# chongkuiqi/S2ANet

Hardware: AMD Instinct MI355X
Metric: 1024x1024 DOTA chips/sec (R-50-FPN S2ANet inference) (higher is better)
Workload: dtype f16; 1 GPU; BASELINE configs[2]: full R-50-FPN S2ANet inference, batch 8 of 1024x1024 synthetic uint8 chips per GPU; 3 independent batches in flight on 3 HIP streams; global_batch=8, num_classes=15, weights=seeded random init of the reference architecture; odm_cls bias calibrated, nms_candidate_cap=160000, nms_candidates_dropped=0, distinct_input_batches=3, fam_cls_branch=True, hip_graph=False, batches_in_flight=3, parallelism=dp1 (one process per GPU)

## Files before the change

include/s2anet_hip.h:

```cpp
#ifndef S2ANET_HIP_H_
#define S2ANET_HIP_H_

#include <stddef.h>
#include <stdint.h>

#ifdef __cplusplus
extern "C" {
#endif

#define S2A_OK 0
#define S2A_EINVAL (-1)
#define S2A_EWORKSPACE (-2)
#define S2A_EHIP (-3)
#define S2A_ENOTIMPL (-4)

#define S2A_DTYPE_F32 0
#define S2A_DTYPE_F16 1
#define S2A_DTYPE_F64 2

#define S2A_LAYOUT_NCHW 0
#define S2A_LAYOUT_NHWC 1

typedef void* s2a_stream_t;

// ... 194 lines not shown
int s2a_deform_conv_backward(int dtype, const void* input, const void* offset, const void* grad_output, const void* weight,
                             float* grad_input_f32, void* grad_offset, float* grad_weight_f32, float scale, int64_t batch,
                             int64_t channels, int64_t height, int64_t width, int64_t out_channels, void* workspace,
                             size_t workspace_bytes, s2a_stream_t stream);
int s2a_deform_conv_backward_typed(int dtype, const void* input, const void* offset, const void* grad_output,
                                   const void* weight, void* grad_input, void* grad_offset, float* grad_weight_f32,
                                   float scale, int64_t batch, int64_t channels, int64_t height, int64_t width,
                                   int64_t out_channels, void* workspace, size_t workspace_bytes, s2a_stream_t stream);

int s2a_conv3x3_tail1x1_f16(const void* x, const void* weight_frag, const void* bias, const void* tail_weight_frag,
                            const void* tail_bias, const void* residual, void* out, const void* chain_weight_frag,
                            const void* chain_bias, void* chain_out, int64_t chain_channels, int64_t batch, int64_t channels,
                            int64_t mid_channels, int64_t out_channels, int64_t height, int64_t width,
                            s2a_stream_t stream);

int s2a_conv1x1_add_up2_f16(const void* x, const void* weight_frag, const void* bias, const void* coarse,
                            void* out, int64_t batch, int64_t channels, int64_t height, int64_t width,
                            int64_t out_channels, s2a_stream_t stream);

int64_t s2a_pyramid_pixels(const s2a_pyramid* pyr, int64_t batch);
int s2a_conv3x3_pyramid_f16(const void* x, const void* weight_frag, const void* bias, const void* residual,
                            void* out, int64_t batch, int64_t channels, int64_t out_channels, int relu,
                            const s2a_pyramid* pyr, s2a_stream_t stream);
int s2a_conv3x3_head_pyramid_f16(const void* x, const void* weight_frag, const void* bias, void* out,
                                 const void* head_weight_frag, const void* head_bias, void* head_out,
                                 int64_t batch, int64_t channels, int64_t out_channels, int relu,
                                 const s2a_pyramid* pyr, s2a_stream_t stream);
int s2a_orconv_pool_pyramid_f16(const void* x, const void* weight_frag, const void* bias, void* out, void* pooled,
                                int64_t batch, int64_t channels, int64_t out_channels, const s2a_pyramid* pyr,
                                s2a_stream_t stream);
int64_t s2a_conv_wino_packed_elems(int64_t out_channels, int64_t channels);
int s2a_conv_wino_pack_weight_f16(const void* weight, int64_t out_channels, int64_t channels, void* packed,
                                  s2a_stream_t stream);
int s2a_conv3x3_wino_pyramid_f16(const void* x, const void* weight_wino, const void* bias, void* out, void* pooled,
                                 int64_t batch, int64_t channels, int64_t out_channels, int relu,
                                 const s2a_pyramid* pyr, s2a_stream_t stream);
int s2a_align_conv_pyramid_f16(const void* x, const float* anchors, const void* weight_packed, void* out,
                               int64_t batch, int64_t channels, int64_t out_channels, int relu,
                               const s2a_pyramid* pyr, s2a_stream_t stream);
int s2a_fam_refine_anchors_pyramid(const void* pred, int64_t row_stride, int64_t batch, const s2a_pyramid* pyr,
                                   float anchor_scale, float* refined, s2a_stream_t stream);

int64_t s2a_stem_packed_elems(void);
int s2a_stem_pack_weight_f16(const void* weight, void* packed, s2a_stream_t stream);
int s2a_stem_u8_f16(const void* image_u8, const void* weight_packed, const void* bias, void* out,
                    int64_t batch, int64_t height, int64_t width, float divisor, s2a_stream_t stream);
// ... 46 lines not shown
```

s2anet_amd/_lib.py:

```python
import ctypes
import os
import subprocess

import torch

_HERE = os.path.dirname(os.path.abspath(__file__))
LIB_PATH = os.environ.get("S2A_LIB_PATH") or os.path.join(_HERE, "libs2anet_hip.so")

OK, EINVAL, EWORKSPACE, EHIP, ENOTIMPL = 0, -1, -2, -3, -4
DTYPE_F32, DTYPE_F16, DTYPE_F64 = 0, 1, 2
LAYOUT_NCHW, LAYOUT_NHWC = 0, 1

c_i64, c_int, c_f32, c_sz, c_vp = (ctypes.c_int64, ctypes.c_int, ctypes.c_float, ctypes.c_size_t,
                                   ctypes.c_void_p)


class DcnParams(ctypes.Structure):
    _fields_ = [("batch", c_i64), ("channels", c_i64), ("height", c_i64), ("width", c_i64),
                ("out_channels", c_i64),
                ("kW", c_int), ("kH", c_int), ("dW", c_int), ("dH", c_int), ("padW", c_int),
                ("padH", c_int), ("dilationW", c_int), ("dilationH", c_int), ("group", c_int),
                ("deformable_group", c_int), ("dtype", c_int), ("offset_dtype", c_int),
                ("layout", c_int), ("relu", c_int)]

# ... 89 lines not shown
    "s2a_deform_conv_backward_weight_workspace_bytes": (c_sz, [c_i64, c_i64, c_i64, c_i64, c_i64]),
    "s2a_deform_conv_backward_workspace_bytes": (c_sz, [c_int, c_i64, c_i64, c_i64, c_i64, c_i64]),
    "s2a_deform_conv_backward": (c_int, [c_int, c_vp, c_vp, c_vp, c_vp, c_vp, c_vp, c_vp, c_f32, c_i64, c_i64, c_i64, c_i64,
                                         c_i64, c_vp, c_sz, c_vp]),
    "s2a_deform_conv_backward_typed": (c_int, [c_int, c_vp, c_vp, c_vp, c_vp, c_vp, c_vp, c_vp, c_f32, c_i64, c_i64, c_i64, c_i64,
                                               c_i64, c_vp, c_sz, c_vp]),
    "s2a_deform_conv_backward_input_f32_workspace_bytes": (c_sz, [c_i64, c_i64, c_i64, c_i64, c_i64]),
    "s2a_deform_conv_backward_weight_f32_workspace_bytes": (c_sz, [c_i64, c_i64, c_i64, c_i64, c_i64]),
    "s2a_deform_conv_backward_weight_f32": (c_int, [c_vp, c_vp, c_vp, c_vp, c_f32, c_i64, c_i64, c_i64, c_i64, c_i64,
                                                    c_vp, c_sz, c_vp]),
    "s2a_deform_conv_backward_input_f32": (c_int, [c_vp, c_vp, c_vp, c_vp, c_vp, c_vp, c_i64, c_i64, c_i64, c_i64, c_i64,
                                                   c_vp, c_sz, c_vp]),
    "s2a_deform_conv_backward_weight_f16": (c_int, [c_vp, c_vp, c_vp, c_vp, c_i64, c_i64, c_i64, c_i64, c_i64, c_vp, c_sz, c_vp]),
    "s2a_deform_conv_backward_input_f16": (c_int, [c_vp, c_vp, c_vp, c_vp, c_vp, c_vp, c_i64, c_i64, c_i64, c_i64, c_i64,
                                           c_vp, c_sz, c_vp]),
    "s2a_deformable_im2col": (c_int, [c_vp, c_vp, c_vp, ctypes.POINTER(DcnParams), c_vp]),
    "s2a_deformable_col2im": (c_int, [c_vp, c_vp, c_vp, ctypes.POINTER(DcnParams), c_vp]),
    "s2a_deformable_col2im_coord": (c_int, [c_vp, c_vp, c_vp, c_vp, ctypes.POINTER(DcnParams), c_vp]),
    "s2a_conv3x3_tail1x1_f16": (c_int, [c_vp] * 10 + [c_i64] * 7 + [c_vp]),
    "s2a_conv1x1_add_up2_f16": (c_int, [c_vp, c_vp, c_vp, c_vp, c_vp, c_i64, c_i64, c_i64, c_i64, c_i64, c_vp]),
    "s2a_pyramid_pixels": (c_i64, [ctypes.POINTER(Pyramid), c_i64]),
    "s2a_conv3x3_pyramid_f16": (c_int, [c_vp, c_vp, c_vp, c_vp, c_vp, c_i64, c_i64, c_i64, c_int,
                                        ctypes.POINTER(Pyramid), c_vp]),
    "s2a_conv3x3_head_pyramid_f16": (c_int, [c_vp, c_vp, c_vp, c_vp, c_vp, c_vp, c_vp, c_i64, c_i64, c_i64, c_int,
                                             ctypes.POINTER(Pyramid), c_vp]),
    "s2a_orconv_pool_pyramid_f16": (c_int, [c_vp, c_vp, c_vp, c_vp, c_vp, c_i64, c_i64, c_i64, ctypes.POINTER(Pyramid), c_vp]),
    "s2a_conv_wino_packed_elems": (c_i64, [c_i64, c_i64]),
    "s2a_conv_wino_pack_weight_f16": (c_int, [c_vp, c_i64, c_i64, c_vp, c_vp]),
    "s2a_conv3x3_wino_pyramid_f16": (c_int, [c_vp, c_vp, c_vp, c_vp, c_vp, c_i64, c_i64, c_i64, c_int,
                                             ctypes.POINTER(Pyramid), c_vp]),
    "s2a_align_conv_pyramid_f16": (c_int, [c_vp, c_vp, c_vp, c_vp, c_i64, c_i64, c_i64, c_int,
                                           ctypes.POINTER(Pyramid), c_vp]),
    "s2a_fam_refine_anchors_pyramid": (c_int, [c_vp, c_i64, c_i64, ctypes.POINTER(Pyramid), c_f32, c_vp, c_vp]),
    "s2a_stem_packed_elems": (c_i64, []),
    "s2a_stem_pack_weight_f16": (c_int, [c_vp, c_vp, c_vp]),
    "s2a_stem_u8_f16": (c_int, [c_vp, c_vp, c_vp, c_vp, c_i64, c_i64, c_i64, c_f32, c_vp]),
    "s2a_pyramid_candidates_count": (c_i64, [ctypes.POINTER(Pyramid), c_i64]),
    "s2a_pyramid_candidates": (c_int, [c_vp, c_vp, c_vp, c_i64, ctypes.POINTER(Pyramid), c_int, c_i64, c_f32, c_vp, c_vp, c_vp, c_vp]),
    "s2a_rbox_to_poly": (c_int, [c_vp, c_i64, c_i64, c_vp, c_vp]),
    "s2a_scene_gather_u8": (c_int, [c_vp, c_i64, c_i64, c_vp, c_i64, ctypes.c_int32, c_vp, c_vp]),
    "s2a_scene_merge_workspace_bytes": (c_sz, [c_i64, c_i64]),
    "s2a_scene_merge": (c_int, [c_vp, c_vp, c_vp, c_vp, c_vp, c_i64, c_i64, ctypes.c_int32, ctypes.c_double, c_i64,
                                c_vp, c_vp, c_vp, c_vp, c_vp, c_vp, c_vp, c_sz, c_vp]),
    "s2a_delta2bbox_rotated": (c_int, [c_vp, c_vp, c_i64, c_f32, c_vp, c_vp]),
    "s2a_fam_refine_anchors": (c_int, [c_vp, c_i64, c_i64, c_i64, c_f32, c_f32, c_int, c_int,
                                       c_vp, c_vp]),
# ... 78 lines not shown
```

s2anet_amd/csrc/dcn_ops.hip:

```cpp
#include <hip/hip_fp16.h>
#include <hip/hip_runtime.h>

#include <algorithm>
#include <cstdlib>
#include <cstring>

#include "common.hpp"

namespace s2a {
namespace {

#ifndef S2A_ABL
#define S2A_ABL 0
#endif
#ifndef S2A_STAMP
#define S2A_STAMP 0
#endif
#ifdef S2A_MEASURE
#define S2A_DCN_DROP_SWITCH(xb, wb)                     \
  do {                                                  \
    const char* drop = getenv("S2A_DCN_DROP");          \
    if (drop && strchr(drop, 'x')) (xb) = 0;            \
    if (drop && strchr(drop, 'w')) (wb) = 0;            \
  } while (0)
// ... 1074 lines not shown
  }
  dcn_patch_tile<OUT_NHWC, SRC, TH>(a.x, a.src, a.wfrag, a.out, a.Ntot, a.C, a.H, a.W, a.O, a.stride, a.relu, a.x_bytes, a.lt,
                                        a.tile_base, blockIdx.x, a.n_full ? a.n_full : gridDim.x, threadIdx.x);
}

constexpr int kCPW = 18;

struct ConvExtra {
  _Float16* pool_out;
  const _Float16* head_w;
  const _Float16* head_b;
  _Float16* head_out;
  int store_main;
  const _Float16* tail_w;
  const _Float16* tail_b;
  const _Float16* tail_res;
  _Float16* tail_out;
  const _Float16* chain_w;
  const _Float16* chain_b;
  _Float16* chain_out;
  int chain_O;
};

template <int TAPS, int OG, int PH = 1, int SD = 1, bool TAIL = false, int HT = 0>
struct ConvCfg {
  static constexpr int kTH = (SD == 2 || HT) ? 4 : 8 * PH;
  static constexpr int kPos = (SD == 2 || HT) ? 64 : 128 * PH;
  static constexpr int kWaves = 4 * PH;
  static constexpr int kPW = SD == 2 ? 33 : kCPW;
  static constexpr int kNT = (kPos / 32) * OG / 4 / PH;
  static constexpr int kPix = TAPS == 9 ? ((kTH - 1) * SD + 3) * kPW : kPos;
  static constexpr int kDma = (kPix * 9 + 63) / 64;
  static constexpr int kPatchBytes = kDma * 1024;
  static constexpr int kOutRowB = OG * 128 + 16;
  static constexpr bool kWLds = PH == 2 && TAPS == 9;
  static constexpr int kWBuf = OG * 8192;
  static constexpr int kLoop0 = 2 * kPatchBytes + (kWLds ? 2 * kWBuf : 0);
  static constexpr int kLoop = (kWLds && OG == 1 && kPatchBytes + 9 * 8192 > kLoop0) ? kPatchBytes + 9 * 8192 : kLoop0;
  static constexpr int kLds0 = (kLoop > kPos * kOutRowB) ? kLoop : kPos * kOutRowB;
  static constexpr int kTailRowB = 528;
  static constexpr int kLds = (TAIL && kPos * kTailRowB > kLds0) ? kPos * kTailRowB : kLds0;
  static constexpr int kBiasBytes = TAIL ? 1024 : 512;
  static constexpr int kJ = (kDma + kWaves - 1) / kWaves;
};

template <int TAPS, int OG, int PH = 1, int SD = 1, bool TAIL = false, int HT = 0>
__global__ __launch_bounds__(256 * PH, PH == 1 ? 2 : 1) void k_conv_f16(const _Float16* __restrict__ x_,
                                                     const _Float16* __restrict__ wfrag,
                                                     const _Float16* __restrict__ bias,
                                                     const _Float16* __restrict__ residual_,
                                                     _Float16* __restrict__ out_, int64_t Ntot_, int C,
                                                     int H_, int W_, int Ho_, int Wo_, int cstride, int O,
                                                     int relu, unsigned x_bytes_, LevelTab lt, int res_up,
                                                     ConvExtra ex) {
  _Float16* pool_out_ = ex.pool_out;
  using T = _Float16;
  using V = f16x8;
  using Cfg = ConvCfg<TAPS, OG, PH, SD, TAIL, HT>;
  constexpr int NT = Cfg::kNT;
  static_assert(NT >= 1, "unsupported tile / group combination");
  static_assert(!HT || (TAPS == 9 && PH == 1 && SD == 1 && !TAIL), "half tiles: plain 3x3 / stride 1");
  static_assert(!TAIL || (TAPS == 9 && OG == 1 && SD == 1), "the fused 1x1 tail follows a 64-map 3x3/s1");
  constexpr int WPG = 4 / OG;
  constexpr int kThreads_ = 256 * PH;
  extern __shared__ __attribute__((aligned(16))) char smem[];
  const int tid = threadIdx.x, lane = tid & 63, wave = tid >> 6;
  const int wave4 = wave & 3, blk = wave >> 2;
  int64_t tile = xcd_remap(blockIdx.x, gridDim.x);
  const T* x = x_;
  const T* residual = residual_;
  T* out = out_;
  int64_t Ntot = Ntot_;
  int H = H_, W = W_, Ho = Ho_, Wo = Wo_;
  unsigned x_bytes = x_bytes_;
  if (TAPS == 9 && lt.n > 1) {
    int t0 = 0, p0 = 0;
#pragma unroll
    for (int i = 0; i < kMaxLevels; i++)
      if (i < lt.n && tile >= lt.tile0[i]) {
        t0 = lt.tile0[i]; p0 = lt.pix0[i]; H = lt.H[i]; W = lt.W[i];
      }
    tile -= t0;
    Ho = H; Wo = W;
    Ntot = (int64_t)lt.batch * H * W;
    x += (int64_t)p0 * C;
// ... 48 lines not shown
  }
  auto patch_issue = [&](int cc) {
    char* P = smem + (cc & 1) * Cfg::kPatchBytes;
#pragma unroll
    for (int j = 0; j < Cfg::kJ; j++) {
      const int i = wave_u + Cfg::kWaves * j;
      if (i < Cfg::kDma)
        __builtin_amdgcn_raw_ptr_buffer_load_lds(rx, (__attribute__((address_space(3))) void*)(P + i * 1024), 16,
                                                 (int)pvoff[j], cc * 128, 0, 0);
    }
  };

  const int grp = wave4 / WPG, sub = wave4 % WPG;
  const bool wave_active = grp * 64 < Oloc;
  const int g = min(o0 / 64 + grp, G - 1);
  const V* wf_base = reinterpret_cast<const V*>(wfrag) + lane;
  V wA[2][4], wB[2][4];
  constexpr bool M16 = (TAPS == 9 && SD == 1) || (TAPS == 1 && OG == 4);
  constexpr int NB16 = 2 * NT;
  auto load_w = [&](int s, V (&wv)[2][4]) {
    if constexpr (M16) {
      const V* p = reinterpret_cast<const V*>(wfrag) + ((int64_t)s * G + g) * 8 * 64 + ((lane >> 4) & 1) * 128 + (lane >> 5) * 32 + (lane & 15);
#pragma unroll
      for (int f = 0; f < 8; f++) wv[f >> 2][f & 3] = p[((f >> 2) * 4 + (f & 1)) * 64 + ((f >> 1) & 1) * 16];
      return;
    }
    const V* p = wf_base + ((int64_t)s * G + g) * 8 * 64;
#pragma unroll
    for (int a = 0; a < 2; a++)
#pragma unroll
      for (int kk = 0; kk < 4; kk++) wv[a][kk] = p[(a * 4 + kk) * 64];
  };
  const int lp = (TAPS == 9 && SD == 1) ? ((lane & 16) | (((lane & 15) - ((lane >> 3) & 2)) & 15)) : (lane & 31);
  int fbase[NT];
#pragma unroll
  for (int b = 0; b < NT; b++) {
    int pl = 128 * blk + 32 * (sub * NT + b) + lp;
    int pix = TAPS == 9 ? SD * ((pl >> 4) * Cfg::kPW + (pl & 15)) : pl;
    fbase[b] = pix * kRowBytes + (lane >> 5) * 16;
  }
  f32x16 acc[2][NT];
  f32x4 acc16[M16 ? 4 : 1][M16 ? NB16 : 1];
  if constexpr (M16) {
#pragma unroll
    for (int a = 0; a < 4; a++)
#pragma unroll
      for (int b = 0; b < NB16; b++)
// ... 5 lines not shown
#pragma unroll
      for (int b = 0; b < NT; b++)
#pragma unroll
        for (int r = 0; r < 16; r++) acc[a][b][r] = 0.f;
  }
  const int kg16 = lane >> 4, i16 = lane & 15;
  const int pix16 = (i16 >= 4 && i16 < 12) ? (((i16 - 4) >> 1) * 4 + (i16 & 1))
                                           : (((i16 & 3) >> 1) * 4 + 2 + (i16 & 1) + (i16 >= 12 ? 8 : 0));
  const int t16 = 2 * sub * NT;
  const int fbase16 = (TAPS == 9 ? (8 * blk + t16) * Cfg::kPW + pix16 : 128 * blk + 16 * t16 + pix16) * kRowBytes + (kg16 & 1) * 64 + (kg16 >> 1) * 16;
  constexpr int kTile16 = (TAPS == 9 ? Cfg::kPW : 16) * kRowBytes;
  const int abase16 = (kg16 & 1) * 2048 + ((kg16 >> 1) * 32 + i16) * 16;

  auto compute = [&](const char* P, int t, const V (&wv)[2][4]) {
    if (!wave_active) return;
    const int toff = ((t / 3) * Cfg::kPW + (t % 3)) * kRowBytes;
    if constexpr (M16) {
#pragma unroll
      for (int ks = 0; ks < 2; ks++) {
        V pf[NB16];
#pragma unroll
        for (int b = 0; b < NB16; b++) pf[b] = *reinterpret_cast<const V*>(P + fbase16 + b * kTile16 + toff + ks * 32);
#pragma unroll
        for (int a = 0; a < 4; a++)
#pragma unroll
          for (int b = 0; b < NB16; b++)
            acc16[a][b] = __builtin_amdgcn_mfma_f32_16x16x32_f16(wv[(a * 2 + ks) >> 2][(a * 2 + ks) & 3], pf[b], acc16[a][b], 0, 0, 0);
      }
      return;
    }
#pragma unroll
    for (int kk = 0; kk < 4; kk++) {
      V pf[NT];
#pragma unroll
      for (int b = 0; b < NT; b++) pf[b] = *reinterpret_cast<const V*>(P + fbase[b] + toff + kk * 32);
#pragma unroll
      for (int a = 0; a < 2; a++)
#pragma unroll
        for (int b = 0; b < NT; b++)
          acc[a][b] = __builtin_amdgcn_mfma_f32_32x32x16_f16(wv[a][kk], pf[b], acc[a][b], 0, 0, 0);
    }
  };

  constexpr bool kEarlyRes = TAIL && Cfg::kWLds;
  constexpr int NI2 = TAIL ? Cfg::kPos * 32 / kThreads_ : 1;
  unsigned off2[NI2];
  V r2[NI2];
  auto tail_res_issue = [&]() {
    const __amdgpu_buffer_rsrc_t rr = __builtin_amdgcn_make_buffer_rsrc(
        const_cast<T*>(ex.tail_res ? ex.tail_res : ex.tail_out), 0, (int)((uint64_t)Ntot * 256 * 2), 0x00020000);
#pragma unroll
    for (int i = 0; i < NI2; i++) {
      const int idx = tid + kThreads_ * i, pos = idx >> 5, col = idx & 31;
      const int64_t gp = tile_pos(tile, pos, Cfg::kTH, Ho, Wo, HWo, Ntot);
      off2[i] = gp >= 0 ? (unsigned)((gp * 256 + col * 8) * 2) : 0x80000000u;
      r2[i] = __builtin_bit_cast(V, __builtin_amdgcn_raw_buffer_load_b128(rr, (int)(ex.tail_res ? off2[i] : 0x80000000u), 0, 0));
    }
  };
  const int nstage = TAPS * CC, last = nstage - 1;
#if S2A_STAMP
  unsigned long long t_tic = 0, t_work = 0, t_wait = 0;
  if ((Cfg::kWLds && OG == 4) || (TAPS == 1 && OG == 4 && SD == 1)) S2A_STAMP_AT(0);
#endif
  if constexpr (Cfg::kWLds) {
    char* wb = smem + 2 * Cfg::kPatchBytes;
    const __amdgpu_buffer_rsrc_t rw = __builtin_amdgcn_make_buffer_rsrc(
        const_cast<T*>(wfrag), 0, (int)((uint64_t)O * (uint64_t)(CC * 64) * 9 * 2), 0x00020000);
    const int wbase = (o0 / 64) * 8192;
    auto w_issue = [&](int s) {
#pragma unroll
      for (int j = 0; j < OG; j++) {
        const int piece = wave_u * OG + j;
        __builtin_amdgcn_raw_ptr_buffer_load_lds(rw, (__attribute__((address_space(3))) void*)(wb + (s & 1) * Cfg::kWBuf + piece * 1024),
                                                 16, piece * 1024 + lane * 16, s * G * 8192 + wbase, 0, 0);
      }
    };
    auto compute_wl = [&](const char* P, int t, const char* Wb) {
      const int toff = ((t / 3) * Cfg::kPW + (t % 3)) * kRowBytes;
      if constexpr (M16) {
#pragma unroll
        for (int ks = 0; ks < 2; ks++) {
          V wv[4], pf[NB16];
#pragma unroll
          for (int a = 0; a < 4; a++)
            wv[a] = *reinterpret_cast<const V*>(Wb + grp * 8192 + abase16 + (a >> 1) * 4096 + ks * 1024 + (a & 1) * 256);
#pragma unroll
          for (int b = 0; b < NB16; b++)
            pf[b] = *reinterpret_cast<const V*>(P + fbase16 + b * kTile16 + toff + ks * 32);
#pragma unroll
          for (int a = 0; a < 4; a++)
#pragma unroll
            for (int b = 0; b < NB16; b++)
              acc16[a][b] = __builtin_amdgcn_mfma_f32_16x16x32_f16(wv[a], pf[b], acc16[a][b], 0, 0, 0);
        }
        return;
// ... 68 lines not shown
  if constexpr (TAPS == 9) {
    for (int cc = 0; cc < CC; cc++) {
      const int s0 = cc * 9;
      const char* Pc = smem + (cc & 1) * Cfg::kPatchBytes;
#define S2A_TAP(T_, WCUR, WNEXT)                                                     \
      load_w(min(s0 + (T_) + 1, last), WNEXT);                                          \
      compute(Pc, (T_), WCUR);                                                          \
      __builtin_amdgcn_sched_barrier(0);
      S2A_TAP(0, wA, wB)
      S2A_TAP(1, wB, wA)
      S2A_TAP(2, wA, wB)
      S2A_TAP(3, wB, wA)
      S2A_TAP(4, wA, wB)
      S2A_TAP(5, wB, wA)
      if (cc + 1 < CC) patch_issue(cc + 1);
      S2A_TAP(6, wA, wB)
      S2A_TAP(7, wB, wA)
      S2A_TAP(8, wA, wB)
#undef S2A_TAP
      __syncthreads();
#pragma unroll
      for (int a = 0; a < 2; a++)
#pragma unroll
        for (int kk = 0; kk < 4; kk++) wA[a][kk] = wB[a][kk];
    }
  } else {
#define S2A_STAGE(C_, WCUR, WNEXT)                                                   \
    if ((C_) + 1 < CC) patch_issue((C_) + 1);                                           \
    load_w(min((C_) + 1, last), WNEXT);                                                 \
    S2A_TIC();                                                                          \
    compute(smem + ((C_) & 1) * Cfg::kPatchBytes, 0, WCUR);                             \
    S2A_TOC(t_work); S2A_TIC();                                                         \
    __syncthreads();                                                                    \
    S2A_TOC(t_wait);
    int cc = 0;
    for (; cc + 1 < CC; cc += 2) {
      S2A_STAGE(cc, wA, wB)
      S2A_STAGE(cc + 1, wB, wA)
    }
    if (cc < CC) { S2A_STAGE(cc, wA, wB) }
#undef S2A_STAGE
#if S2A_STAMP
    if (TAPS == 1 && OG == 4 && SD == 1) { S2A_STAMP_AT(3); S2A_STAMP_VAL(6, t_work); S2A_STAMP_VAL(7, t_wait); }
#endif
  }
  }

// ... 866 lines not shown
int build_flags_dcn() {
  int f = S2A_ABL & 0xff;
  if (S2A_STAMP) f |= 1 << 9;
#ifdef S2A_MEASURE
  f |= 1 << 10;
#endif
  return f;
}
}

extern "C" int s2a_debug_read_stamps(unsigned long long* host_dst, int64_t count) {
#if S2A_STAMP
  S2A_HIP(hipMemcpyFromSymbol(host_dst, HIP_SYMBOL(s2a::g_stamps), (size_t)count * 8));
  return S2A_OK;
#else
  (void)host_dst; (void)count;
  s2a::set_error("s2a_debug_read_stamps: not a diagnostic build");
  return S2A_ENOTIMPL;
#endif
}

namespace s2a {
namespace {
template <int TAPS, int OG, int PH = 1, int SD = 1, bool TAIL = false, int HT = 0>
int launch_conv(const _Float16* x, const _Float16* wfrag, const _Float16* bias, const _Float16* residual,
                _Float16* out, int64_t B, int C, int H, int W, int Ho, int Wo, int cstride, int O, int relu,
                hipStream_t st, const LevelTab* levels = nullptr, int64_t level_tiles = 0, int res_up = 0,
                ConvExtra ex = ConvExtra{nullptr, nullptr, nullptr, nullptr, 1}) {
  using Cfg = ConvCfg<TAPS, OG, PH, SD, TAIL, HT>;
  const int64_t Ntot = B * (int64_t)Ho * Wo;
  int64_t tiles = TAPS == 9 ? B * ((Wo + 15) / 16) * ((Ho + Cfg::kTH - 1) / Cfg::kTH) : (Ntot + Cfg::kPos - 1) / Cfg::kPos;
  LevelTab lt = {};
  if (levels) { lt = *levels; tiles = level_tiles; }
  dim3 grid((unsigned)tiles, (unsigned)((O + 64 * OG - 1) / (64 * OG)));
  auto kern = k_conv_f16<TAPS, OG, PH, SD, TAIL, HT>;
  S2A_HIP(hipFuncSetAttribute(reinterpret_cast<const void*>(kern), hipFuncAttributeMaxDynamicSharedMemorySize, Cfg::kLds + Cfg::kBiasBytes));
  kern<<<grid, 256 * PH, Cfg::kLds + Cfg::kBiasBytes, st>>>(x, wfrag, bias, residual, out, Ntot, C, H, W, Ho, Wo, cstride, O, relu,
                                     (unsigned)((uint64_t)B * H * W * C * 2), lt, res_up, ex);
  S2A_LAUNCH_CHECK();
  return S2A_OK;
}
}
}

extern "C" int s2a_conv_nhwc_f16(const void* x, const void* weight_frag, const void* bias, const void* residual,
                                 void* out, int64_t batch, int64_t channels, int64_t height, int64_t width,
                                 int64_t out_channels, int ksize, int stride, int relu, s2a_stream_t stream) {
  S2A_CHECK_ARG(batch >= 0 && channels > 0 && out_channels > 0 && height > 0 && width > 0, "conv: bad shape");
  S2A_CHECK_ARG(ksize == 3 || ksize == 1, "conv: kernel size must be 1 or 3");
  S2A_CHECK_ARG(stride == 1 || stride == 2, "conv: stride must be 1 or 2");
  S2A_CHECK_ARG(!(ksize == 3 && stride == 2) || out_channels % 128 == 0, "conv: 3x3 stride 2 needs out_channels % 128 == 0");
  S2A_CHECK_ARG((channels % 64 == 0 || channels == 32) && out_channels % 64 == 0,
                "conv: channels must be 32 or a multiple of 64, out_channels a multiple of 64");
  const uint64_t x_bytes = (uint64_t)batch * height * width * channels * 2;
  S2A_CHECK_ARG(x_bytes < (1ull << 31) && (ksize == 1 || (height < 32000 && width < 32000)),
                "conv: input too large for 32-bit offsets");
  S2A_CHECK_ARG(!residual || (uint64_t)batch * ((height - 1) / stride + 1) * ((width - 1) / stride + 1) * out_channels * 2 < (1ull << 31),
                "conv: output too large for the fused residual (32-bit offsets)");
  if (batch == 0) return S2A_OK;
  S2A_CHECK_ARG(x && weight_frag && out, "conv: NULL tensor");
  S2A_CHECK_ARG(((uintptr_t)x % 16) == 0 && ((uintptr_t)out % 16) == 0 && ((uintptr_t)weight_frag % 16) == 0 &&
                ((uintptr_t)bias % 8) == 0 && ((uintptr_t)residual % 16) == 0, "conv: tensors must be 16-byte aligned");
  hipStream_t st = as_stream(stream);
  const int Ho = (int)((height - 1) / stride + 1), Wo = (int)((width - 1) / stride + 1);
  const int og = out_channels % 256 == 0 ? 4 : (out_channels % 128 == 0 ? 2 : 1);
  const _Float16 *X = (const _Float16*)x, *Wf = (const _Float16*)weight_frag, *Bi = (const _Float16*)bias,
                 *R = (const _Float16*)residual;
  _Float16* Y = (_Float16*)out;
#define S2A_CONV(TAPS, OG_) launch_conv<TAPS, OG_>(X, Wf, Bi, R, Y, batch, (int)channels, (int)height, (int)width, Ho, Wo, stride, (int)out_channels, relu, st)
  if (ksize == 3 && stride == 2) {
    if (og == 4)
      return launch_conv<9, 4, 1, 2>(X, Wf, Bi, R, Y, batch, (int)channels, (int)height, (int)width, Ho, Wo, 2,
                                     (int)out_channels, relu, st);
    return launch_conv<9, 2, 1, 2>(X, Wf, Bi, R, Y, batch, (int)channels, (int)height, (int)width, Ho, Wo, 2,
                                   (int)out_channels, relu, st);
  }
  if (ksize == 3 && og < 4 && channels % 64 == 0) {
    const int64_t tiles16 = batch * ((Wo + 15) / 16) * ((Ho + 15) / 16) * ((out_channels + 64 * og - 1) / (64 * og));
    int ph = tiles16 >= 256 ? 2 : 1;
    if (const char* f = getenv("S2A_CONV_PH_NARROW")) ph = atoi(f) == 2 ? 2 : 1;
    if (ph == 2) {
      if (og == 2)
        return launch_conv<9, 2, 2>(X, Wf, Bi, R, Y, batch, (int)channels, (int)height, (int)width, Ho, Wo, 1,
                                    (int)out_channels, relu, st);
      return launch_conv<9, 1, 2>(X, Wf, Bi, R, Y, batch, (int)channels, (int)height, (int)width, Ho, Wo, 1,
                                  (int)out_channels, relu, st);
    }
  }
  if (ksize == 3 && og == 4 && channels % 64 == 0) {
    const int64_t tiles16 = batch * ((Wo + 15) / 16) * ((Ho + 15) / 16) * (out_channels / 256);
    int ph = tiles16 >= 512 ? 2 : 1;
    if (const char* f = getenv("S2A_CONV_PH")) ph = atoi(f) == 2 ? 2 : 1;
    if (ph == 2)
      return launch_conv<9, 4, 2>(X, Wf, Bi, R, Y, batch, (int)channels, (int)height, (int)width, Ho, Wo, 1,
                                  (int)out_channels, relu, st);
  }
// ... 117 lines not shown
  int64_t tiles = 0, pix = 0;
  for (int i = 0; i < pyr->n_levels; i++) {
    const int64_t H = pyr->height[i], W = pyr->width[i];
    if (H < 1 || W < 1 || H >= 32000 || W >= 32000) return -1;
    lt->H[i] = (int)H; lt->W[i] = (int)W; lt->stride[i] = pyr->stride[i];
    lt->tile0[i] = (int)tiles; lt->pix0[i] = (int)pix;
    tiles += batch * ((W + 15) / 16) * ((H + tile_rows - 1) / tile_rows);
    pix += batch * H * W;
    if (tiles >= (1ll << 31) || pix >= (1ll << 31)) return -1;
  }
  *total_pix = pix;
  return tiles;
}
}
}

extern "C" int64_t s2a_pyramid_pixels(const s2a_pyramid* pyr, int64_t batch) {
  LevelTab lt; int64_t pix = 0;
  return build_levels(pyr, batch, &lt, &pix) < 0 ? -1 : pix;
}

static int conv3x3_pyramid_impl(const void* x, const void* weight_frag, const void* bias, const void* residual,
                                void* out, ConvExtra ex, int64_t batch, int64_t channels, int64_t out_channels,
                                int relu, const s2a_pyramid* pyr, s2a_stream_t stream);

extern "C" int s2a_conv3x3_pyramid_f16(const void* x, const void* weight_frag, const void* bias, const void* residual,
                                       void* out, int64_t batch, int64_t channels, int64_t out_channels,
                                       int relu, const s2a_pyramid* pyr, s2a_stream_t stream) {
  return conv3x3_pyramid_impl(x, weight_frag, bias, residual, out, ConvExtra{nullptr, nullptr, nullptr, nullptr, 1}, batch,
                              channels, out_channels, relu, pyr, stream);
}

extern "C" int s2a_conv3x3_head_pyramid_f16(const void* x, const void* weight_frag, const void* bias, void* out,
                                            const void* head_weight_frag, const void* head_bias, void* head_out,
                                            int64_t batch, int64_t channels, int64_t out_channels, int relu,
                                            const s2a_pyramid* pyr, s2a_stream_t stream) {
  S2A_CHECK_ARG(out_channels == 256, "conv3x3_head_pyramid: the fused 1x1 head needs a 256-channel tower");
  S2A_CHECK_ARG(head_weight_frag && head_bias && head_out, "conv3x3_head_pyramid: NULL head tensor");
  S2A_CHECK_ARG(((uintptr_t)head_weight_frag % 16) == 0 && ((uintptr_t)head_bias % 8) == 0 && ((uintptr_t)head_out % 16) == 0,
                "conv3x3_head_pyramid: misaligned head tensor");
  ConvExtra ex{nullptr, (const _Float16*)head_weight_frag, (const _Float16*)head_bias, (_Float16*)head_out, out != nullptr};
  return conv3x3_pyramid_impl(x, weight_frag, bias, nullptr, out ? out : head_out, ex, batch, channels, out_channels, relu,
                              pyr, stream);
}

extern "C" int s2a_orconv_pool_pyramid_f16(const void* x, const void* weight_frag, const void* bias, void* out,
                                           void* pooled, int64_t batch, int64_t channels, int64_t out_channels,
                                           const s2a_pyramid* pyr, s2a_stream_t stream) {
  S2A_CHECK_ARG(pooled != nullptr && ((uintptr_t)pooled % 16) == 0 && out_channels % 64 == 0,
                "orconv_pool_pyramid: pooled must be a 16-byte aligned buffer, out_channels a multiple of 64");
  return conv3x3_pyramid_impl(x, weight_frag, bias, nullptr, out, ConvExtra{(_Float16*)pooled, nullptr, nullptr, nullptr, 1},
                              batch, channels, out_channels, 0, pyr, stream);
}

static int conv3x3_pyramid_impl(const void* x, const void* weight_frag, const void* bias, const void* residual,
                                void* out, ConvExtra ex, int64_t batch, int64_t channels, int64_t out_channels,
                                int relu, const s2a_pyramid* pyr, s2a_stream_t stream) {
  S2A_CHECK_ARG(batch >= 0 && channels > 0 && out_channels > 0, "conv_pyramid: bad shape");
  S2A_CHECK_ARG((channels % 64 == 0 || channels == 32) && out_channels % 64 == 0,
                "conv_pyramid: channels must be 32 or a multiple of 64, out_channels a multiple of 64");
  LevelTab lt; int64_t pix = 0;
  int og = out_channels % 256 == 0 ? 4 : (out_channels % 128 == 0 ? 2 : 1);
  const char* og_env = getenv("S2A_CONV_OG");
  if (og_env && !ex.head_w) og = std::min(og, std::max(1, atoi(og_env)));
  int ph = (og == 4 && channels % 64 == 0) ? 2 : 1;
  if (const char* f = getenv("S2A_CONV_PH")) ph = atoi(f) == 2 && og == 4 && channels % 64 == 0 ? 2 : 1;
  const int64_t tiles = build_levels(pyr, batch, &lt, &pix, 8 * ph);
  S2A_CHECK_ARG(tiles >= 0, "conv_pyramid: bad level table (1..8 levels, positive sizes)");
  S2A_CHECK_ARG((uint64_t)pix * channels * 2 < (1ull << 31), "conv_pyramid: input too large for 32-bit offsets");
  if (batch == 0) return S2A_OK;
  S2A_CHECK_ARG(x && weight_frag && out, "conv_pyramid: NULL tensor");
  S2A_CHECK_ARG(((uintptr_t)x % 16) == 0 && ((uintptr_t)out % 16) == 0 && ((uintptr_t)weight_frag % 16) == 0 &&
                ((uintptr_t)bias % 8) == 0 && ((uintptr_t)residual % 16) == 0, "conv_pyramid: tensors must be 16-byte aligned");
  if (lt.n == 1) lt.n = 2, lt.tile0[1] = 0x7fffffff;
  hipStream_t st = as_stream(stream);
  const _Float16 *X = (const _Float16*)x, *Wf = (const _Float16*)weight_frag, *Bi = (const _Float16*)bias,
                 *R = (const _Float16*)residual;
  _Float16* Y = (_Float16*)out;
  const ConvExtra Pq = ex;
#define S2A_CONVP(OG_) launch_conv<9, OG_>(X, Wf, Bi, R, Y, batch, (int)channels, lt.H[0], lt.W[0], lt.H[0], lt.W[0], 1, (int)out_channels, relu, st, &lt, tiles, 0, Pq)
  if (ph == 2 && og == 4)
    return launch_conv<9, 4, 2>(X, Wf, Bi, R, Y, batch, (int)channels, lt.H[0], lt.W[0], lt.H[0], lt.W[0], 1,
                                (int)out_channels, relu, st, &lt, tiles, 0, Pq);
  return og == 4 ? S2A_CONVP(4) : (og == 2 ? S2A_CONVP(2) : S2A_CONVP(1));
#undef S2A_CONVP
}

extern "C" int s2a_align_conv_pyramid_f16(const void* x, const float* anchors, const void* weight_packed, void* out,
                                          int64_t batch, int64_t channels, int64_t out_channels, int relu,
                                          const s2a_pyramid* pyr, s2a_stream_t stream) {
  S2A_CHECK_ARG(batch >= 0 && channels > 0 && out_channels > 0, "align_conv_pyramid: bad shape");
  S2A_CHECK_ARG(channels % 64 == 0 && out_channels % 64 == 0, "align_conv_pyramid: channels and out_channels must be multiples of 64");
  LevelTab lt; int64_t pix = 0;
  const int64_t tiles = build_levels(pyr, batch, &lt, &pix);
  S2A_CHECK_ARG(tiles >= 0, "align_conv_pyramid: bad level table (1..8 levels, positive sizes)");
  for (int i = 0; i < lt.n; i++) {
    S2A_CHECK_ARG(lt.stride[i] > 0, "align_conv: stride must be positive");
    S2A_CHECK_ARG(lt.H[i] >= 3 && lt.W[i] >= 3, "input image is smaller than kernel");
  }
  S2A_CHECK_ARG((uint64_t)pix * channels * 2 < (1ull << 31), "align_conv_pyramid: input too large for 32-bit offsets");
  if (batch == 0) return S2A_OK;
  S2A_CHECK_ARG(x && anchors && weight_packed && out, "align_conv_pyramid: NULL tensor");
  S2A_CHECK_ARG(((uintptr_t)x % 16) == 0 && ((uintptr_t)out % 16) == 0 && ((uintptr_t)weight_packed % 16) == 0,
                "align_conv_pyramid: tensors must be 16-byte aligned");
  if (lt.n == 1) lt.n = 2, lt.tile0[1] = 0x7fffffff;
  hipStream_t st = as_stream(stream);
  const _Float16* wfrag = (const _Float16*)weight_packed + (size_t)out_channels * channels * 9;
// ... 20 lines not shown
```

s2anet_amd/fused.py:

```python
import torch
import torch.nn as nn
import torch.nn.functional as F

from . import _lib


def bias_act_(y, bias, residual=None, relu=False, out=None):
    _lib.require_cuda(y, bias, residual)
    B, C, H, W = y.shape
    if out is not None:
        assert out.shape == y.shape and out.dtype == y.dtype and out.permute(0, 2, 3, 1).is_contiguous()
    ok = (y.is_contiguous(memory_format=torch.channels_last) and
          C % (8 if y.dtype == torch.float16 else 4) == 0 and y.dtype in (torch.float16, torch.float32) and
          (residual is None or (residual.shape == y.shape and residual.dtype == y.dtype and
                                residual.is_contiguous(memory_format=torch.channels_last))))
    if not ok:
        y = y + bias.view(1, -1, 1, 1).to(y.dtype)
        if residual is not None:
            y = y + residual
        y = F.relu(y) if relu else y
        return y if out is None else out.copy_(y)
    b = bias if bias.dtype == y.dtype and bias.is_contiguous() else bias.to(y.dtype).contiguous()
    with torch.cuda.device(y.device):
        _lib.check(_lib.lib().s2a_bias_act_nhwc_to(_lib.ptr(y), _lib.ptr(b), _lib.ptr(residual),
# ... 7 lines not shown
    if not (x.is_cuda and x.dtype == torch.float16 and x.dim() == 4 and
            x.is_contiguous(memory_format=torch.channels_last) and tuple(dilation) == (1, 1) and groups == 1 and
            (in_channels % 64 == 0 or in_channels == 32) and (out_channels % 64 == 0 or out_channels < 64) and
            x.numel() * 2 < (1 << 31)):
        return False
    if os.environ.get("S2A_NO_OWN_CONV"):
        return False
    k, st, pd = tuple(kernel_size), tuple(stride), tuple(padding)
    B, _, H, W = x.shape
    narrow = out_channels < 64 or bool(os.environ.get("S2A_OWN_CONV_ALWAYS"))
    if k == (3, 3) and st == (1, 1) and pd == (1, 1):
        return narrow or B * ((H + 7) // 8) * ((W + 15) // 16) >= 64
    if k == (3, 3) and st == (2, 2) and pd == (1, 1) and not os.environ.get("S2A_NO_OWN_CONV_S2"):
        Ho, Wo = (H - 1) // 2 + 1, (W - 1) // 2 + 1
        return out_channels % 128 == 0 and in_channels % 64 == 0 and (narrow or B * ((Ho + 3) // 4) * ((Wo + 15) // 16) >= 128)
    if k == (1, 1) and pd == (0, 0) and st in ((1, 1), (2, 2)) and not os.environ.get("S2A_NO_OWN_CONV1"):
        Ho, Wo = (H - 1) // st[0] + 1, (W - 1) // st[1] + 1
        return narrow or B * Ho * Wo >= 64 * 128
    return False


def conv_pack_weight(weight):
    w = weight.detach().to(torch.float16).contiguous()
    if w.shape[0] < 64:
        w = torch.cat([w, w.new_zeros((64 - w.shape[0],) + tuple(w.shape[1:]))], 0).contiguous()
    if w.shape[1] == 32:
        w = torch.cat([w, torch.zeros_like(w)], 1).contiguous()
    out = torch.empty_like(w)
    with torch.cuda.device(w.device):
        _lib.check(_lib.lib().s2a_conv_pack_weight_f16(_lib.ptr(w), w.shape[0], w.shape[1], w.shape[2],
                                                       _lib.ptr(out), _lib.stream_ptr(w.device)))
    return out


def conv_wino_pack_weight(weight):
    w = weight.detach().to(torch.float16).contiguous()
    O, C = w.shape[:2]
    assert tuple(w.shape[2:]) == (3, 3) and O % 64 == 0 and C % 32 == 0
    L = _lib.lib()
    out = torch.empty((L.s2a_conv_wino_packed_elems(O, C),), dtype=torch.float16, device=w.device)
    with torch.cuda.device(w.device):
        _lib.check(L.s2a_conv_wino_pack_weight_f16(_lib.ptr(w), O, C, _lib.ptr(out), _lib.stream_ptr(w.device)))
    return out


def conv_wino_f16(x, packed_wino, bias, out_channels, relu=False, pool=False):
    from .pyramid import PyramidLayout, conv3x3_wino
    B, C, H, W = x.shape
    assert x.dtype == torch.float16 and x.is_contiguous(memory_format=torch.channels_last)
    lay = PyramidLayout(B, [(H, W)], [1.0])
    b = None if bias is None else bias.to(torch.float16).contiguous()
    r = conv3x3_wino(lay, x.permute(0, 2, 3, 1).reshape(-1, C), packed_wino, b, out_channels, relu, pool)
    if pool:
        return (r[0].view(B, H, W, out_channels).permute(0, 3, 1, 2), r[1].view(B, H, W, out_channels // 8).permute(0, 3, 1, 2))
# ... 206 lines not shown
```

s2anet_amd/pyramid.py:

```python
import ctypes

import torch

from . import _lib


class PyramidLayout:

    def __init__(self, batch, sizes, strides):
        assert 1 <= len(sizes) <= 8 and len(sizes) == len(strides)
        self.batch, self.sizes, self.strides = int(batch), [tuple(map(int, s)) for s in sizes], list(strides)
        self.c = _lib.Pyramid()
        self.c.n_levels = len(sizes)
        self.pix0, p = [], 0
        for i, ((h, w), s) in enumerate(zip(self.sizes, strides)):
            self.c.height[i], self.c.width[i], self.c.stride[i] = h, w, float(s)
            self.pix0.append(p)
            p += self.batch * h * w
        self.pixels = p

    def key(self):
        return (self.batch, tuple(self.sizes), tuple(self.strides))

    def new(self, channels, device, dtype=torch.float16):
        return torch.empty((self.pixels, channels), dtype=dtype, device=device)

    def level(self, buf, l, channels=None):
        h, w = self.sizes[l]
        v = buf[self.pix0[l]:self.pix0[l] + self.batch * h * w].view(self.batch, h, w, buf.shape[1])
        if channels is not None:
            v = v[..., :channels]
        return v.permute(0, 3, 1, 2)

    def rows(self, buf, l):
        h, w = self.sizes[l]
        return buf[self.pix0[l]:self.pix0[l] + self.batch * h * w]


def conv3x3(layout, x, packed_w, bias, out_channels, relu, residual=None, out=None):
    L = _lib.lib()
    if out is None:
        out = layout.new(out_channels, x.device)
    with torch.cuda.device(x.device):
        _lib.check(L.s2a_conv3x3_pyramid_f16(_lib.ptr(x), _lib.ptr(packed_w), _lib.ptr(bias), _lib.ptr(residual),
                                             _lib.ptr(out), layout.batch, x.shape[1], out_channels, int(bool(relu)),
                                             ctypes.byref(layout.c), _lib.stream_ptr(x.device)))
    return out


def conv3x3_head(layout, x, packed_w, bias, out_channels, head_w, head_b, relu=True, keep_tower=False):
    L = _lib.lib()
    head_out = layout.new(64, x.device)
    tower = layout.new(out_channels, x.device) if keep_tower else None
    with torch.cuda.device(x.device):
        _lib.check(L.s2a_conv3x3_head_pyramid_f16(_lib.ptr(x), _lib.ptr(packed_w), _lib.ptr(bias), _lib.ptr(tower), _lib.ptr(head_w),
                                                  _lib.ptr(head_b), _lib.ptr(head_out), layout.batch, x.shape[1], out_channels,
                                                  int(bool(relu)), ctypes.byref(layout.c), _lib.stream_ptr(x.device)))
    return (head_out, tower) if keep_tower else head_out


def orconv_pool(layout, x, packed_w, bias, out_channels, n_orientation=8):
    assert n_orientation == 8
    L = _lib.lib()
    out = layout.new(out_channels, x.device)
    pooled = layout.new(out_channels // 8, x.device)
    with torch.cuda.device(x.device):
# ... 76 lines not shown
```

Measured before the change: 1901 chips/s.

## Skip padded output-channel MFMAs in head convs and stage stride-2 filters via LDS

```diff
diff --git a/include/s2anet_hip.h b/include/s2anet_hip.h
--- a/include/s2anet_hip.h
+++ b/include/s2anet_hip.h
@@ -240,6 +240,9 @@
 int s2a_conv3x3_pyramid_f16(const void* x, const void* weight_frag, const void* bias, const void* residual,
                             void* out, int64_t batch, int64_t channels, int64_t out_channels, int relu,
                             const s2a_pyramid* pyr, s2a_stream_t stream);
+int s2a_conv3x3_pyramid_live_f16(const void* x, const void* weight_frag, const void* bias, const void* residual,
+                                 void* out, int64_t batch, int64_t channels, int64_t out_channels,
+                                 int64_t live_out_channels, int relu, const s2a_pyramid* pyr, s2a_stream_t stream);
 int s2a_conv3x3_head_pyramid_f16(const void* x, const void* weight_frag, const void* bias, void* out,
                                  const void* head_weight_frag, const void* head_bias, void* head_out,
                                  int64_t batch, int64_t channels, int64_t out_channels, int relu,
diff --git a/s2anet_amd/_lib.py b/s2anet_amd/_lib.py
--- a/s2anet_amd/_lib.py
+++ b/s2anet_amd/_lib.py
@@ -135,6 +135,8 @@
     "s2a_pyramid_pixels": (c_i64, [ctypes.POINTER(Pyramid), c_i64]),
     "s2a_conv3x3_pyramid_f16": (c_int, [c_vp, c_vp, c_vp, c_vp, c_vp, c_i64, c_i64, c_i64, c_int,
                                         ctypes.POINTER(Pyramid), c_vp]),
+    "s2a_conv3x3_pyramid_live_f16": (c_int, [c_vp, c_vp, c_vp, c_vp, c_vp, c_i64, c_i64, c_i64, c_i64, c_int,
+                                             ctypes.POINTER(Pyramid), c_vp]),
     "s2a_conv3x3_head_pyramid_f16": (c_int, [c_vp, c_vp, c_vp, c_vp, c_vp, c_vp, c_vp, c_i64, c_i64, c_i64, c_int,
                                              ctypes.POINTER(Pyramid), c_vp]),
     "s2a_orconv_pool_pyramid_f16": (c_int, [c_vp, c_vp, c_vp, c_vp, c_vp, c_i64, c_i64, c_i64, ctypes.POINTER(Pyramid), c_vp]),
diff --git a/s2anet_amd/csrc/dcn_ops.hip b/s2anet_amd/csrc/dcn_ops.hip
--- a/s2anet_amd/csrc/dcn_ops.hip
+++ b/s2anet_amd/csrc/dcn_ops.hip
@@ -1120,7 +1120,7 @@
   int chain_O;
 };
 
-template <int TAPS, int OG, int PH = 1, int SD = 1, bool TAIL = false, int HT = 0>
+template <int TAPS, int OG, int PH = 1, int SD = 1, bool TAIL = false, int HT = 0, int WL = 0>
 struct ConvCfg {
   static constexpr int kTH = (SD == 2 || HT) ? 4 : 8 * PH;
   static constexpr int kPos = (SD == 2 || HT) ? 64 : 128 * PH;
@@ -1131,7 +1131,7 @@
   static constexpr int kDma = (kPix * 9 + 63) / 64;
   static constexpr int kPatchBytes = kDma * 1024;
   static constexpr int kOutRowB = OG * 128 + 16;
-  static constexpr bool kWLds = PH == 2 && TAPS == 9;
+  static constexpr bool kWLds = (PH == 2 && TAPS == 9) || WL;
   static constexpr int kWBuf = OG * 8192;
   static constexpr int kLoop0 = 2 * kPatchBytes + (kWLds ? 2 * kWBuf : 0);
   static constexpr int kLoop = (kWLds && OG == 1 && kPatchBytes + 9 * 8192 > kLoop0) ? kPatchBytes + 9 * 8192 : kLoop0;
@@ -1142,7 +1142,7 @@
   static constexpr int kJ = (kDma + kWaves - 1) / kWaves;
 };
 
-template <int TAPS, int OG, int PH = 1, int SD = 1, bool TAIL = false, int HT = 0>
+template <int TAPS, int OG, int PH = 1, int SD = 1, bool TAIL = false, int HT = 0, int LT = 0, int WL = 0>
 __global__ __launch_bounds__(256 * PH, PH == 1 ? 2 : 1) void k_conv_f16(const _Float16* __restrict__ x_,
                                                      const _Float16* __restrict__ wfrag,
                                                      const _Float16* __restrict__ bias,
@@ -1154,11 +1154,16 @@
   _Float16* pool_out_ = ex.pool_out;
   using T = _Float16;
   using V = f16x8;
-  using Cfg = ConvCfg<TAPS, OG, PH, SD, TAIL, HT>;
+  using Cfg = ConvCfg<TAPS, OG, PH, SD, TAIL, HT, WL>;
   constexpr int NT = Cfg::kNT;
   static_assert(NT >= 1, "unsupported tile / group combination");
   static_assert(!HT || (TAPS == 9 && PH == 1 && SD == 1 && !TAIL), "half tiles: plain 3x3 / stride 1");
   static_assert(!TAIL || (TAPS == 9 && OG == 1 && SD == 1), "the fused 1x1 tail follows a 64-map 3x3/s1");
+  static_assert(LT == 0 || (LT <= 2 && TAPS == 9 && OG == 1 && PH == 1 && SD == 1 && !TAIL && !HT),
+                "live tiles: the plain 8 x 16 form of a 64-column 3x3 / stride 1");
+  static_assert(!WL || (TAPS == 9 && OG == 2 && PH == 1 && SD == 2 && !TAIL && !HT && !LT),
+                "filter through LDS on four waves: the 128-column 3x3 / stride 2");
+  constexpr int NA = LT ? LT : 4;
   constexpr int WPG = 4 / OG;
   constexpr int kThreads_ = 256 * PH;
   extern __shared__ __attribute__((aligned(16))) char smem[];
@@ -1253,7 +1258,7 @@
     if constexpr (M16) {
       const V* p = reinterpret_cast<const V*>(wfrag) + ((int64_t)s * G + g) * 8 * 64 + ((lane >> 4) & 1) * 128 + (lane >> 5) * 32 + (lane & 15);
 #pragma unroll
-      for (int f = 0; f < 8; f++) wv[f >> 2][f & 3] = p[((f >> 2) * 4 + (f & 1)) * 64 + ((f >> 1) & 1) * 16];
+      for (int f = 0; f < 2 * NA; f++) wv[f >> 2][f & 3] = p[((f >> 2) * 4 + (f & 1)) * 64 + ((f >> 1) & 1) * 16];
       return;
     }
     const V* p = wf_base + ((int64_t)s * G + g) * 8 * 64;
@@ -1305,7 +1310,7 @@
 #pragma unroll
         for (int b = 0; b < NB16; b++) pf[b] = *reinterpret_cast<const V*>(P + fbase16 + b * kTile16 + toff + ks * 32);
 #pragma unroll
-        for (int a = 0; a < 4; a++)
+        for (int a = 0; a < NA; a++)
 #pragma unroll
           for (int b = 0; b < NB16; b++)
             acc16[a][b] = __builtin_amdgcn_mfma_f32_16x16x32_f16(wv[(a * 2 + ks) >> 2][(a * 2 + ks) & 3], pf[b], acc16[a][b], 0, 0, 0);
@@ -1350,10 +1355,11 @@
     const __amdgpu_buffer_rsrc_t rw = __builtin_amdgcn_make_buffer_rsrc(
         const_cast<T*>(wfrag), 0, (int)((uint64_t)O * (uint64_t)(CC * 64) * 9 * 2), 0x00020000);
     const int wbase = (o0 / 64) * 8192;
+    constexpr int kWJ = 8 * OG / Cfg::kWaves;
     auto w_issue = [&](int s) {
 #pragma unroll
-      for (int j = 0; j < OG; j++) {
-        const int piece = wave_u * OG + j;
+      for (int j = 0; j < kWJ; j++) {
+        const int piece = wave_u * kWJ + j;
         __builtin_amdgcn_raw_ptr_buffer_load_lds(rw, (__attribute__((address_space(3))) void*)(wb + (s & 1) * Cfg::kWBuf + piece * 1024),
                                                  16, piece * 1024 + lane * 16, s * G * 8192 + wbase, 0, 0);
       }
@@ -1468,7 +1474,8 @@
 #pragma unroll
       for (int a = 0; a < 2; a++)
 #pragma unroll
-        for (int kk = 0; kk < 4; kk++) wA[a][kk] = wB[a][kk];
+        for (int kk = 0; kk < 4; kk++)
+          if (a * 4 + kk < 2 * NA) wA[a][kk] = wB[a][kk];
     }
   } else {
 #define S2A_STAGE(C_, WCUR, WNEXT)                                                   \
@@ -2381,18 +2388,18 @@
 
 namespace s2a {
 namespace {
-template <int TAPS, int OG, int PH = 1, int SD = 1, bool TAIL = false, int HT = 0>
+template <int TAPS, int OG, int PH = 1, int SD = 1, bool TAIL = false, int HT = 0, int LT = 0, int WL = 0>
 int launch_conv(const _Float16* x, const _Float16* wfrag, const _Float16* bias, const _Float16* residual,
                 _Float16* out, int64_t B, int C, int H, int W, int Ho, int Wo, int cstride, int O, int relu,
                 hipStream_t st, const LevelTab* levels = nullptr, int64_t level_tiles = 0, int res_up = 0,
                 ConvExtra ex = ConvExtra{nullptr, nullptr, nullptr, nullptr, 1}) {
-  using Cfg = ConvCfg<TAPS, OG, PH, SD, TAIL, HT>;
+  using Cfg = ConvCfg<TAPS, OG, PH, SD, TAIL, HT, WL>;
   const int64_t Ntot = B * (int64_t)Ho * Wo;
   int64_t tiles = TAPS == 9 ? B * ((Wo + 15) / 16) * ((Ho + Cfg::kTH - 1) / Cfg::kTH) : (Ntot + Cfg::kPos - 1) / Cfg::kPos;
   LevelTab lt = {};
   if (levels) { lt = *levels; tiles = level_tiles; }
   dim3 grid((unsigned)tiles, (unsigned)((O + 64 * OG - 1) / (64 * OG)));
-  auto kern = k_conv_f16<TAPS, OG, PH, SD, TAIL, HT>;
+  auto kern = k_conv_f16<TAPS, OG, PH, SD, TAIL, HT, LT, WL>;
   S2A_HIP(hipFuncSetAttribute(reinterpret_cast<const void*>(kern), hipFuncAttributeMaxDynamicSharedMemorySize, Cfg::kLds + Cfg::kBiasBytes));
   kern<<<grid, 256 * PH, Cfg::kLds + Cfg::kBiasBytes, st>>>(x, wfrag, bias, residual, out, Ntot, C, H, W, Ho, Wo, cstride, O, relu,
                                      (unsigned)((uint64_t)B * H * W * C * 2), lt, res_up, ex);
@@ -2431,6 +2438,11 @@
     if (og == 4)
       return launch_conv<9, 4, 1, 2>(X, Wf, Bi, R, Y, batch, (int)channels, (int)height, (int)width, Ho, Wo, 2,
                                      (int)out_channels, relu, st);
+    bool wl = true;
+    if (const char* f = getenv("S2A_CONV_S2_WLDS")) wl = atoi(f) != 0;
+    if (wl)
+      return launch_conv<9, 2, 1, 2, false, 0, 0, 1>(X, Wf, Bi, R, Y, batch, (int)channels, (int)height, (int)width, Ho, Wo, 2,
+                                                     (int)out_channels, relu, st);
     return launch_conv<9, 2, 1, 2>(X, Wf, Bi, R, Y, batch, (int)channels, (int)height, (int)width, Ho, Wo, 2,
                                    (int)out_channels, relu, st);
   }
@@ -2594,13 +2606,23 @@
 
 static int conv3x3_pyramid_impl(const void* x, const void* weight_frag, const void* bias, const void* residual,
                                 void* out, ConvExtra ex, int64_t batch, int64_t channels, int64_t out_channels,
-                                int relu, const s2a_pyramid* pyr, s2a_stream_t stream);
+                                int relu, const s2a_pyramid* pyr, s2a_stream_t stream, int64_t live = 0);
 
 extern "C" int s2a_conv3x3_pyramid_f16(const void* x, const void* weight_frag, const void* bias, const void* residual,
                                        void* out, int64_t batch, int64_t channels, int64_t out_channels,
                                        int relu, const s2a_pyramid* pyr, s2a_stream_t stream) {
   return conv3x3_pyramid_impl(x, weight_frag, bias, residual, out, ConvExtra{nullptr, nullptr, nullptr, nullptr, 1}, batch,
                               channels, out_channels, relu, pyr, stream);
+}
+
+extern "C" int s2a_conv3x3_pyramid_live_f16(const void* x, const void* weight_frag, const void* bias, const void* residual,
+                                            void* out, int64_t batch, int64_t channels, int64_t out_channels,
+                                            int64_t live_out_channels, int relu, const s2a_pyramid* pyr,
+                                            s2a_stream_t stream) {
+  S2A_CHECK_ARG(live_out_channels >= 1 && live_out_channels <= out_channels,
+                "conv_pyramid_live: live_out_channels must be in 1..out_channels");
+  return conv3x3_pyramid_impl(x, weight_frag, bias, residual, out, ConvExtra{nullptr, nullptr, nullptr, nullptr, 1}, batch,
+                              channels, out_channels, relu, pyr, stream, live_out_channels);
 }
 
 extern "C" int s2a_conv3x3_head_pyramid_f16(const void* x, const void* weight_frag, const void* bias, void* out,
@@ -2627,7 +2649,7 @@
 
 static int conv3x3_pyramid_impl(const void* x, const void* weight_frag, const void* bias, const void* residual,
                                 void* out, ConvExtra ex, int64_t batch, int64_t channels, int64_t out_channels,
-                                int relu, const s2a_pyramid* pyr, s2a_stream_t stream) {
+                                int relu, const s2a_pyramid* pyr, s2a_stream_t stream, int64_t live) {
   S2A_CHECK_ARG(batch >= 0 && channels > 0 && out_channels > 0, "conv_pyramid: bad shape");
   S2A_CHECK_ARG((channels % 64 == 0 || channels == 32) && out_channels % 64 == 0,
                 "conv_pyramid: channels must be 32 or a multiple of 64, out_channels a multiple of 64");
@@ -2650,11 +2672,16 @@
                  *R = (const _Float16*)residual;
   _Float16* Y = (_Float16*)out;
   const ConvExtra Pq = ex;
-#define S2A_CONVP(OG_) launch_conv<9, OG_>(X, Wf, Bi, R, Y, batch, (int)channels, lt.H[0], lt.W[0], lt.H[0], lt.W[0], 1, (int)out_channels, relu, st, &lt, tiles, 0, Pq)
+#define S2A_CONVP(OG_, LT_) launch_conv<9, OG_, 1, 1, false, 0, LT_>(X, Wf, Bi, R, Y, batch, (int)channels, lt.H[0], lt.W[0], lt.H[0], lt.W[0], 1, (int)out_channels, relu, st, &lt, tiles, 0, Pq)
   if (ph == 2 && og == 4)
     return launch_conv<9, 4, 2>(X, Wf, Bi, R, Y, batch, (int)channels, lt.H[0], lt.W[0], lt.H[0], lt.W[0], 1,
                                 (int)out_channels, relu, st, &lt, tiles, 0, Pq);
-  return og == 4 ? S2A_CONVP(4) : (og == 2 ? S2A_CONVP(2) : S2A_CONVP(1));
+  if (out_channels == 64 && live > 0 && live <= 32) {
+    bool on = true;
+    if (const char* f = getenv("S2A_CONV_LIVE")) on = atoi(f) != 0;
+    if (on) return live <= 16 ? S2A_CONVP(1, 1) : S2A_CONVP(1, 2);
+  }
+  return og == 4 ? S2A_CONVP(4, 0) : (og == 2 ? S2A_CONVP(2, 0) : S2A_CONVP(1, 0));
 #undef S2A_CONVP
 }
 
diff --git a/s2anet_amd/fused.py b/s2anet_amd/fused.py
--- a/s2anet_amd/fused.py
+++ b/s2anet_amd/fused.py
@@ -53,6 +53,7 @@
 
 def conv_pack_weight(weight):
     w = weight.detach().to(torch.float16).contiguous()
+    live = w.shape[0]
     if w.shape[0] < 64:
         w = torch.cat([w, w.new_zeros((64 - w.shape[0],) + tuple(w.shape[1:]))], 0).contiguous()
     if w.shape[1] == 32:
@@ -61,6 +62,8 @@
     with torch.cuda.device(w.device):
         _lib.check(_lib.lib().s2a_conv_pack_weight_f16(_lib.ptr(w), w.shape[0], w.shape[1], w.shape[2],
                                                        _lib.ptr(out), _lib.stream_ptr(w.device)))
+    if live < out.shape[0]:
+        out.live_out_channels = live
     return out
 
 
diff --git a/s2anet_amd/pyramid.py b/s2anet_amd/pyramid.py
--- a/s2anet_amd/pyramid.py
+++ b/s2anet_amd/pyramid.py
@@ -41,7 +41,13 @@
     L = _lib.lib()
     if out is None:
         out = layout.new(out_channels, x.device)
+    live = getattr(packed_w, "live_out_channels", None)
     with torch.cuda.device(x.device):
+        if live is not None and live < out_channels:
+            _lib.check(L.s2a_conv3x3_pyramid_live_f16(_lib.ptr(x), _lib.ptr(packed_w), _lib.ptr(bias), _lib.ptr(residual),
+                                                      _lib.ptr(out), layout.batch, x.shape[1], out_channels, int(live),
+                                                      int(bool(relu)), ctypes.byref(layout.c), _lib.stream_ptr(x.device)))
+            return out
         _lib.check(L.s2a_conv3x3_pyramid_f16(_lib.ptr(x), _lib.ptr(packed_w), _lib.ptr(bias), _lib.ptr(residual),
                                              _lib.ptr(out), layout.batch, x.shape[1], out_channels, int(bool(relu)),
                                              ctypes.byref(layout.c), _lib.stream_ptr(x.device)))
```

After: 1897 chips/s, median of 2. Within noise of the previous version (-0.2%).
